# Siverteh/semantic-slam-master

Measured on AMD Instinct MI355X. Metric: frames/sec extract+match on TUM 640x480; match-index bit-exact vs CPU ref, higher is better.
Workload: dtype f32

## Files before the change

semantic-slam-master_amd/csrc/match.hip:

```cpp
#include "common.h"

namespace {

constexpr int QB = 128;
constexpr int CB = 64;
constexpr int NTM = 256;

template <int ROWS, int D>
struct Stager {
    static constexpr int GL = D == 128 ? 4 : 5, GM = D / 8 - 1, LDD = D + 4;
    static constexpr int ITEMS = ROWS * (D / 8) / NTM;
    float4 lo[ITEMS], hi[ITEMS];
    bool ok[ITEMS];
    __device__ __forceinline__ void load(const float *__restrict__ src, int first, int n_valid, int tid) {
#pragma unroll
        for (int i = 0; i < ITEMS; i++) {
            const int it = tid + NTM * i, row = it >> GL, g = it & GM;
            ok[i] = first + row < n_valid;
            const float4 *p = reinterpret_cast<const float4 *>(src + (long long)(ok[i] ? first + row : 0) * D + 8 * g);
            lo[i] = p[0];
            hi[i] = p[1];
        }
    }
    __device__ __forceinline__ void store(float *dst, int tid) const {
#pragma unroll
        for (int i = 0; i < ITEMS; i++) {
            const int it = tid + NTM * i, row = it >> GL, g = it & GM;
            float4 ev, od;
            const bool k = ok[i];
            kp8_split(make_float4(k ? lo[i].x : 0.f, k ? lo[i].y : 0.f, k ? lo[i].z : 0.f, k ? lo[i].w : 0.f),
                      make_float4(k ? hi[i].x : 0.f, k ? hi[i].y : 0.f, k ? hi[i].z : 0.f, k ? hi[i].w : 0.f), ev, od);
            *reinterpret_cast<float4 *>(dst + row * LDD + 8 * g) = ev;
            *reinterpret_cast<float4 *>(dst + row * LDD + 8 * g + 4) = od;
        }
    }
};

__device__ __forceinline__ unsigned long long sim_key(float v, float qoff, unsigned nqi) {
    unsigned u = __float_as_uint(v + qoff);
    u ^= (unsigned)((int)u >> 31) | 0x80000000u;
    return ((unsigned long long)u << 32) | nqi;
}

struct RowBest {
    float best, second;
    int besti, li;
};
template <int STEP, int CT, bool ONEPASS, bool MASKED, bool SECOND>
__device__ __forceinline__ void red_step(const f32x16 &acc, int sbase, int nc, int r, int h, float qoff, unsigned nqi, RowBest &rb,
                                         unsigned long long (&k)[8], unsigned long long &kk, int &jj) {
    if constexpr (STEP < 8) {
        if constexpr (STEP == 0 && CT == 0) rb.li = -1;
#pragma unroll
        for (int e = 2 * STEP; e < 2 * STEP + 2; e++) {
            const int lit = 32 * CT + (e & 3) + 8 * (e >> 2);
            float v = acc[e];
            if constexpr (MASKED) v = sbase + lit + 4 * h < nc ? v : -INFINITY;
            const bool gt = v > rb.best;
            if constexpr (SECOND) rb.second = __builtin_amdgcn_fmed3f(v, rb.best, rb.second);
            rb.li = gt ? lit : rb.li;
            rb.best = gt ? v : rb.best;
        }
        if constexpr (STEP == 7 && CT == 1) rb.besti = rb.li >= 0 ? sbase + 4 * h + rb.li : rb.besti;
    } else if constexpr (!ONEPASS) {
    } else if constexpr (STEP < 16) {
        constexpr int i = STEP - 8;
        typedef unsigned u32x2 __attribute__((ext_vector_type(2)));
        const unsigned long long lo = sim_key(acc[i], qoff, nqi), hi = sim_key(acc[i + 8], qoff, nqi);
        const u32x2 w0 = __builtin_amdgcn_permlane16_swap((unsigned)lo, (unsigned)hi, false, false);
        const u32x2 w1 = __builtin_amdgcn_permlane16_swap((unsigned)(lo >> 32), (unsigned)(hi >> 32), false, false);
        const unsigned long long a = ((unsigned long long)w1[0] << 32) | w0[0], b = ((unsigned long long)w1[1] << 32) | w0[1];
        k[i] = a > b ? a : b;
    } else if constexpr (STEP < 23) {
        constexpr int m = STEP < 20 ? 4 : (STEP < 22 ? 2 : 1);
        constexpr int i = STEP < 20 ? STEP - 16 : (STEP < 22 ? STEP - 20 : 0);
        const bool up = (r & (2 * m)) != 0;
        unsigned long long lo = k[i], hi = k[i + m];
        asm("" : "+v"(lo), "+v"(hi));
        const unsigned long long keep = up ? hi : lo, send = up ? lo : hi;
        const unsigned long long o = __shfl_xor(send, 2 * m);
        k[i] = keep > o ? keep : o;
    } else {
        const unsigned long long o = __shfl_xor(k[0], 1);
        kk = k[0] > o ? k[0] : o;
        jj = sbase + 32 * CT + crow((r >> 1) & 15, h);
    }
}
template <int FIRST, int N, bool ONEPASS, bool MASKED, bool SECOND>
__device__ __forceinline__ void red_steps(const f32x16 (&acc)[2], int s, int nc, int r, int h, float qoff, unsigned nqi, RowBest &rb,
                                          unsigned long long (&k)[2][8], unsigned long long (&kk)[2], int (&jj)[2]) {
    if constexpr (N > 0) {
        constexpr int ct = FIRST / 24;
        red_step<FIRST % 24, ct, ONEPASS, MASKED, SECOND>(acc[ct], s * CB, nc, r, h, qoff, nqi, rb, k[ct], kk[ct], jj[ct]);
        red_steps<FIRST + 1, N - 1, ONEPASS, MASKED, SECOND>(acc, s, nc, r, h, qoff, nqi, rb, k, kk, jj);
    }
}

struct StridedPairs {
    __device__ __forceinline__ bool frames(long long p, long long &f1, long long &f2) const {
        f1 = f2 = p;
        return true;
    }
    static __device__ __forceinline__ bool unwritten(unsigned long long) { return false; }
};
struct ListedPairs {
    const int *first, *second;
    int n_bank;
    __device__ __forceinline__ bool frames(long long p, long long &f1, long long &f2) const {
        const int a = first[p], b = second[p];
        if ((unsigned)a >= (unsigned)n_bank || (unsigned)b >= (unsigned)n_bank) return false;
        f1 = a;
        f2 = b;
        return true;
    }
    static __device__ __forceinline__ bool unwritten(unsigned long long key) { return key == 0ull; }
};

template <int D, bool ONEPASS, bool SECOND, class PAIRS>
__global__ __launch_bounds__(NTM, D == 128 ? 2 : 1) void sim_argmax_kernel(const float *__restrict__ desc1, long long stride1, int n1,
                                                            const float *__restrict__ desc2, long long stride2, int n2,
                                                            int *__restrict__ nn12, float *__restrict__ s12,
                                                            int *__restrict__ nn21, float *__restrict__ s21,
                                                            float *__restrict__ second12,
                                                            unsigned long long *__restrict__ keys, int n_pairs, int qblocks,
                                                            PAIRS pairs) {
    constexpr int LDD = D + 4;
    __shared__ __attribute__((aligned(16))) float Cs[2 * CB * LDD];
    const int tid = threadIdx.x, lane = tid & 63, wave = tid >> 6, r = lane & 31, h = lane >> 5;
    const int dir = blockIdx.y;
    const int xcd = blockIdx.x & 7, slot = blockIdx.x >> 3;
    const long long pair = (long long)(slot / qblocks) * 8 + xcd;
    if (pair >= n_pairs) return;
    long long f1, f2;
    if (!pairs.frames(pair, f1, f2)) {
        const int i = (slot % qblocks) * QB + tid;
        if (tid < QB && i < (dir == 0 ? n1 : n2)) {
            (dir == 0 ? nn12 + pair * n1 : nn21 + pair * n2)[i] = 0;
            float *val = dir == 0 ? s12 : s21;
            if (val) val[pair * (dir == 0 ? n1 : n2) + i] = 0.0f;
            if (dir == 0 && second12) second12[pair * n1 + i] = 0.0f;
        }
        return;
    }
    const float *q = dir == 0 ? desc1 + f1 * stride1 : desc2 + f2 * stride2;
    const float *c = dir == 0 ? desc2 + f2 * stride2 : desc1 + f1 * stride1;
    const int nq = dir == 0 ? n1 : n2, nc = dir == 0 ? n2 : n1;
    const int q0 = (slot % qblocks) * QB;
    if (q0 >= nq) return;
    int *o_idx = (dir == 0 ? nn12 + pair * n1 : nn21 + pair * n2);
    float *o_val = dir == 0 ? (s12 ? s12 + pair * n1 : nullptr) : (s21 ? s21 + pair * n2 : nullptr);
    float *o_sec = (dir == 0 && second12) ? second12 + pair * n1 : nullptr;

    Stager<CB, D> sc;
    sc.load(c, 0, nc, tid);
    const int qi = q0 + wave * 32 + r;
    const bool qok = qi < nq;
    float qreg[D / 2];
    {
        const float4 *qp = reinterpret_cast<const float4 *>(q + (long long)(qok ? qi : 0) * D);
        const float qm = qok ? 1.0f : 0.0f;
#pragma unroll
        for (int i = 0; i < D / 4; i++) {
            const float4 v = qp[i];
            qreg[2 * i] = (h ? v.y : v.x) * qm;
            qreg[2 * i + 1] = (h ? v.w : v.z) * qm;
        }
    }
    sc.store(Cs, tid);
    __syncthreads();

    RowBest rb = {-INFINITY, -INFINITY, 0x7fffffff, -1};
    const float qoff = qok ? 0.0f : -INFINITY;
    const unsigned nqi = ~(unsigned)qi;
    const int nstage = (nc + CB - 1) / CB;

#define M1_MMA(g_, A_, acc_)                                                                                          \
    {                                                                                                                 \
                    \
        const f32x4 a0 = *reinterpret_cast<const f32x4 *>((A_) + 8 * (g_));                                          \
        const f32x4 a1 = *reinterpret_cast<const f32x4 *>((A_) + 32 * LDD + 8 * (g_));                                \
        _Pragma("unroll") for (int st = 0; st < 4; st++) {                                                            \
            acc_[0] = mfma32(a0[st], qreg[4 * (g_) + st], acc_[0]);                                                   \
            acc_[1] = mfma32(a1[st], qreg[4 * (g_) + st], acc_[1]);                                                   \
        }                                                                                                             \
    }
    auto commit = [&](const unsigned long long (&kk)[2], const int (&jj)[2]) {
        if (ONEPASS) {
#pragma unroll
            for (int ct = 0; ct < 2; ct++)
                if (!(r & 1) && jj[ct] < nc) atomicMax(keys + pair * n2 + jj[ct], kk[ct]);
        }
    };

    f32x16 held[2];
#pragma unroll
    for (int e = 0; e < 16; e++) held[0][e] = held[1][e] = 0.0f;
    {
        const float *A = Cs + r * LDD + 4 * h;
#pragma unroll
        for (int g = 0; g < D / 8; g++) M1_MMA(g, A, held)
    }
    if (nstage > 1) {
        sc.load(c, CB, nc, tid);
        sc.store(Cs + CB * LDD, tid);
    }
    __syncthreads();
    unsigned long long kq[2][8];
    for (int s = 1; s < nstage; s++) {
        if (s + 1 < nstage) sc.load(c, (s + 1) * CB, nc, tid);
        const float *A = Cs + (s & 1) * CB * LDD + r * LDD + 4 * h;
        f32x16 acc[2];
        unsigned long long kk[2] = {0ull, 0ull};
        int jj[2] = {0, 0};
#pragma unroll
        for (int e = 0; e < 16; e++) acc[0][e] = acc[1][e] = 0.0f;
#define M1_SLOT(g_)                                                                                                   \
        _Pragma("unroll") for (int u = 0; u < D / 128; u++) M1_MMA((D / 128) * (g_) + u, A, acc)                       \
        __builtin_amdgcn_sched_barrier(0);                                                                            \
        red_steps<3 * (g_), 3, ONEPASS, false, SECOND>(held, s - 1, nc, r, h, qoff, nqi, rb, kq, kk, jj);                              \
        __builtin_amdgcn_sched_barrier(0);
        M1_SLOT(0) M1_SLOT(1) M1_SLOT(2) M1_SLOT(3) M1_SLOT(4) M1_SLOT(5) M1_SLOT(6) M1_SLOT(7)
        M1_SLOT(8) M1_SLOT(9) M1_SLOT(10) M1_SLOT(11) M1_SLOT(12) M1_SLOT(13) M1_SLOT(14) M1_SLOT(15)
#undef M1_SLOT
        held[0] = acc[0];
        held[1] = acc[1];
        if (s + 1 < nstage) sc.store(Cs + ((s + 1) & 1) * CB * LDD, tid);
        __builtin_amdgcn_sched_barrier(0);
        commit(kk, jj);
        __syncthreads();
    }
#undef M1_MMA
    {
        unsigned long long kk[2] = {0ull, 0ull};
        int jj[2] = {0, 0};
        red_steps<0, 48, ONEPASS, true, SECOND>(held, nstage - 1, nc, r, h, qoff, nqi, rb, kq, kk, jj);
        commit(kk, jj);
    }
    float best = rb.best, second = rb.second;
    int besti = rb.besti;
    {
        const float ov = __shfl_xor(best, 32), os = __shfl_xor(second, 32);
        const int oi = __shfl_xor(besti, 32);
        if (ov > best || (ov == best && oi < besti)) {
            second = fmaxf(best, os);
            best = ov;
            besti = oi;
        } else {
            second = fmaxf(second, ov);
        }
    }
    if (h == 0 && qok) {
        o_idx[qi] = (unsigned)besti < (unsigned)nc ? besti : 0;
        if (o_val) o_val[qi] = best;
        if (o_sec) o_sec[qi] = second;
    }
}

template <class PAIRS>
__global__ __launch_bounds__(256) void keys_decode_kernel(const unsigned long long *__restrict__ keys, long long n, int n1,
                                                           int *__restrict__ nn21, float *__restrict__ s21) {
    const long long i = (long long)blockIdx.x * 256 + threadIdx.x;
    if (i >= n) return;
    const unsigned long long kk = keys[i];
    if (PAIRS::unwritten(kk)) {
        nn21[i] = 0;
        if (s21) s21[i] = 0.0f;
        return;
    }
    unsigned u = (unsigned)(kk >> 32);
    u ^= (u >> 31) ? 0x80000000u : 0xffffffffu;
    const unsigned qi = ~(unsigned)kk;
    nn21[i] = qi < (unsigned)n1 ? (int)qi : 0;
    if (s21) s21[i] = __uint_as_float(u);
}

template <class PAIRS>
__global__ __launch_bounds__(256) void match_finalize_kernel(const int *__restrict__ nn12, const float *__restrict__ s12,
                                                              const int *__restrict__ nn21, int n1, int n2,
                                                              const float *__restrict__ sc1, long long ss1,
                                                              const float *__restrict__ sc2, long long ss2,
                                                              const float *__restrict__ in1, const float *__restrict__ in2,
                                                              float w_desc, float w_sal, float t_sal, float t_sim,
                                                              float t_int, long long *__restrict__ matches,
                                                              float *__restrict__ quality, int *__restrict__ count, PAIRS pairs) {
    __shared__ int wave_tot[4];
    __shared__ int running;
    const int tid = threadIdx.x, lane = tid & 63, wave = tid >> 6;
    const long long p = blockIdx.x;
    long long f1, f2;
    if (!pairs.frames(p, f1, f2)) {
        if (tid == 0) count[p] = 0;
        for (int sl = tid; sl < n1; sl += 256) {
            matches[(p * n1 + sl) * 2] = 0;
            matches[(p * n1 + sl) * 2 + 1] = 0;
            quality[p * n1 + sl] = 0.f;
        }
        return;
    }
    nn12 += p * n1;
    s12 += p * n1;
    nn21 += p * n2;
    sc1 += f1 * ss1;
    sc2 += f2 * ss2;
    if (in1) in1 += f1 * ss1;
    if (in2) in2 += f2 * ss2;
    matches += p * n1 * 2;
    quality += p * n1;
    if (tid == 0) running = 0;
    __syncthreads();
    for (int base = 0; base < n1; base += 256) {
        const int i = base + tid;
        bool ok = false;
        int j = 0;
        float sim = 0.f, avg = 0.f;
        if (i < n1) {
            j = nn12[i];
            if ((unsigned)j < (unsigned)n2 && nn21[j] == i) {
                sim = s12[i];
                avg = (sc1[i] + sc2[j]) / 2.0f;
                ok = (avg >= t_sal) && (sim >= t_sim);
                if (in1 && in2) ok = ok && ((in1[i] + in2[j]) / 2.0f >= t_int);
            }
        }
        int inc = ok ? 1 : 0;
#pragma unroll
        for (int off = 1; off < 64; off <<= 1) {
            const int t = __shfl_up(inc, off);
            if (lane >= off) inc += t;
        }
        if (lane == 63) wave_tot[wave] = inc;
        __syncthreads();
        int off0 = running;
        for (int w = 0; w < wave; w++) off0 += wave_tot[w];
        if (ok) {
            const int slot = off0 + inc - 1;
            matches[2 * slot] = i;
            matches[2 * slot + 1] = j;
            quality[slot] = w_desc * sim + w_sal * avg;
        }
        __syncthreads();
        if (tid == 0) running += wave_tot[0] + wave_tot[1] + wave_tot[2] + wave_tot[3];
        __syncthreads();
    }
    if (tid == 0) count[p] = running;
    for (int sl = running + tid; sl < n1; sl += 256) {
        matches[2 * sl] = 0;
        matches[2 * sl + 1] = 0;
        quality[sl] = 0.f;
    }
}

template <class PAIRS>
__global__ __launch_bounds__(256) void match_finalize_rule_kernel(const int *__restrict__ nn12, const float *__restrict__ s12,
                                                                   const float *__restrict__ second12, const int *__restrict__ nn21,
                                                                   int n1, int n2, int rule, float param,
                                                                   long long *__restrict__ matches, float *__restrict__ value,
                                                                   int *__restrict__ count, PAIRS pairs) {
    __shared__ int wave_tot[4];
    __shared__ int running;
    const int tid = threadIdx.x, lane = tid & 63, wave = tid >> 6;
    const long long p = blockIdx.x;
    long long f1, f2;
    if (!pairs.frames(p, f1, f2)) {
        if (tid == 0) count[p] = 0;
        for (int sl = tid; sl < n1; sl += 256) {
            matches[(p * n1 + sl) * 2] = 0;
            matches[(p * n1 + sl) * 2 + 1] = 0;
            value[p * n1 + sl] = 0.f;
        }
        return;
    }
    nn12 += p * n1;
    s12 += p * n1;
    if (second12) second12 += p * n1;
    if (nn21) nn21 += p * n2;
    matches += p * n1 * 2;
    value += p * n1;
    if (tid == 0) running = 0;
    __syncthreads();
    for (int base = 0; base < n1; base += 256) {
        const int i = base + tid;
        bool ok = false;
        int j = 0;
        float val = 0.f;
        if (i < n1) {
            j = nn12[i];
            if ((unsigned)j < (unsigned)n2) {
                const float best = s12[i];
                if (rule == SSLAM_RULE_TRACKED) {
                    ok = best > param;
                    val = best;
                } else if (nn21[j] == i) {
                    const float sec = second12[i];
                    if (rule == SSLAM_RULE_RATIO_BEST) {
                        ok = best > fmaxf(sec, -1.0f) * param;
                        val = best;
                    } else {
                        ok = __fdiv_rn(sec, __fadd_rn(best, 1e-8f)) < param;
                        val = __fsub_rn(1.0f, best);
                    }
                }
            }
        }
        int inc = ok ? 1 : 0;
#pragma unroll
        for (int off = 1; off < 64; off <<= 1) {
            const int t = __shfl_up(inc, off);
            if (lane >= off) inc += t;
        }
        if (lane == 63) wave_tot[wave] = inc;
        __syncthreads();
        int off0 = running;
        for (int w = 0; w < wave; w++) off0 += wave_tot[w];
        if (ok) {
            const int slot = off0 + inc - 1;
            matches[2 * slot] = i;
            matches[2 * slot + 1] = j;
            value[slot] = val;
        }
        __syncthreads();
        if (tid == 0) running += wave_tot[0] + wave_tot[1] + wave_tot[2] + wave_tot[3];
        __syncthreads();
    }
    if (tid == 0) count[p] = running;
    for (int sl = running + tid; sl < n1; sl += 256) {
        matches[2 * sl] = 0;
        matches[2 * sl + 1] = 0;
        value[sl] = 0.f;
    }
}

}

extern "C" long long sslam_sim_argmax_workspace_bytes(int n2, int n_pairs) {
    if (n2 <= 0 || n_pairs <= 0) return SSLAM_E_INVALID;
    const int forced = (int)sslam_knob(KNOB_M1_VARIANT, 0);
    if (forced == 1 || (forced == 0 && n_pairs < 16)) return 0;
    return (long long)n_pairs * n2 * (long long)sizeof(unsigned long long);
}

template <int D, class PAIRS>
static int launch_sim_argmax(const float *desc1, long long stride1, int n1, const float *desc2, long long stride2, int n2, int n_pairs,
                             int32_t *nn12, float *s12, int32_t *nn21, float *s21, float *second12, void *workspace,
                             long long workspace_bytes, void *stream, PAIRS pairs) {
    if ((long long)n_pairs * ((((n1 > n2 ? n1 : n2) + QB - 1) / QB)) > 0x7ffffff0LL / 8) return SSLAM_E_UNSUPPORTED;
    const int forced = (int)sslam_knob(KNOB_M1_VARIANT, 0);
    hipStream_t st = (hipStream_t)stream;
    const long long need = (long long)n_pairs * n2 * (long long)sizeof(unsigned long long);
    const bool have_ws = workspace && workspace_bytes >= need;
    if (forced == 2 && !have_ws) return SSLAM_E_INVALID;
    if (have_ws && (forced == 2 || (forced == 0 && n_pairs >= 16))) {
        unsigned long long *keys = (unsigned long long *)workspace;
        if (hipMemsetAsync(keys, 0, (size_t)need, st) != hipSuccess) return SSLAM_E_LAUNCH;
        const int qb1 = (n1 + QB - 1) / QB;
        const dim3 grid((unsigned)((n_pairs + 7) / 8 * 8 * qb1), 1, 1);
        if (second12)
            hipLaunchKernelGGL((sim_argmax_kernel<D, true, true, PAIRS>), grid, dim3(NTM), 0, st, desc1, stride1, n1, desc2, stride2, n2, nn12,
                               s12, nn21, s21, second12, keys, n_pairs, qb1, pairs);
        else
            hipLaunchKernelGGL((sim_argmax_kernel<D, true, false, PAIRS>), grid, dim3(NTM), 0, st, desc1, stride1, n1, desc2, stride2, n2, nn12,
                               s12, nn21, s21, second12, keys, n_pairs, qb1, pairs);
        SSLAM_CHECK_LAUNCH();
        const long long n = (long long)n_pairs * n2;
        hipLaunchKernelGGL(keys_decode_kernel<PAIRS>, dim3((unsigned)((n + 255) / 256)), dim3(256), 0, st, keys, n, n1, nn21, s21);
        SSLAM_CHECK_LAUNCH();
        return SSLAM_OK;
    }
    const int nmax = n1 > n2 ? n1 : n2;
    const int qbm = (nmax + QB - 1) / QB;
    const dim3 grid((unsigned)((n_pairs + 7) / 8 * 8 * qbm), 2, 1);
    if (second12)
        hipLaunchKernelGGL((sim_argmax_kernel<D, false, true, PAIRS>), grid, dim3(NTM), 0, st, desc1, stride1, n1, desc2, stride2, n2, nn12, s12,
                           nn21, s21, second12, nullptr, n_pairs, qbm, pairs);
    else
        hipLaunchKernelGGL((sim_argmax_kernel<D, false, false, PAIRS>), grid, dim3(NTM), 0, st, desc1, stride1, n1, desc2, stride2, n2, nn12, s12,
                           nn21, s21, second12, nullptr, n_pairs, qbm, pairs);
    SSLAM_CHECK_LAUNCH();
    return SSLAM_OK;
}

#define SSLAM_BY_WIDTH(d_, call128_, call256_) ((d_) == 128 ? (call128_) : (d_) == 256 ? (call256_) : SSLAM_E_UNSUPPORTED)

extern "C" int sslam_sim_argmax_ws_d(const float *desc1, long long stride1, int n1, const float *desc2, long long stride2,
                                     int n2, int n_pairs, int32_t *nn12, float *s12, int32_t *nn21, float *s21, float *second12,
                                     void *workspace, long long workspace_bytes, int d, void *stream) {
    if (!desc1 || !desc2 || !nn12 || !nn21 || n1 <= 0 || n2 <= 0 || n_pairs <= 0) return SSLAM_E_INVALID;
    if (((uintptr_t)desc1 | (uintptr_t)desc2) & 15 || (stride1 & 3) || (stride2 & 3) || ((uintptr_t)workspace & 7)) return SSLAM_E_INVALID;
    if (sslam_misaligned(4, nn12, s12, nn21, s21, second12)) return SSLAM_E_INVALID;
    return SSLAM_BY_WIDTH(d,
                          launch_sim_argmax<128>(desc1, stride1, n1, desc2, stride2, n2, n_pairs, nn12, s12, nn21, s21, second12, workspace,
                                                 workspace_bytes, stream, StridedPairs{}),
                          launch_sim_argmax<256>(desc1, stride1, n1, desc2, stride2, n2, n_pairs, nn12, s12, nn21, s21, second12, workspace,
                                                 workspace_bytes, stream, StridedPairs{}));
}
extern "C" int sslam_sim_argmax_ws(const float *desc1, long long stride1, int n1, const float *desc2, long long stride2,
                                   int n2, int n_pairs, int32_t *nn12, float *s12, int32_t *nn21, float *s21, float *second12,
                                   void *workspace, long long workspace_bytes, void *stream) {
    return sslam_sim_argmax_ws_d(desc1, stride1, n1, desc2, stride2, n2, n_pairs, nn12, s12, nn21, s21, second12, workspace,
                                 workspace_bytes, SSLAM_D, stream);
}

extern "C" int sslam_sim_argmax_pairs_d(const float *bank, long long frame_stride, int n_bank, int K, const int32_t *pair_first,
                                        const int32_t *pair_second, int n_pairs, int32_t *nn12, float *s12, int32_t *nn21, float *s21,
                                        float *second12, void *workspace, long long workspace_bytes, int d, void *stream) {
    if (!bank || !pair_first || !pair_second || !nn12 || !nn21 || n_bank <= 0 || K <= 0 || n_pairs <= 0) return SSLAM_E_INVALID;
    if (((uintptr_t)bank & 15) || (frame_stride & 3) || ((uintptr_t)workspace & 7) || (((uintptr_t)pair_first | (uintptr_t)pair_second) & 3))
        return SSLAM_E_INVALID;
    if (sslam_misaligned(4, nn12, s12, nn21, s21, second12)) return SSLAM_E_INVALID;
    const ListedPairs lp{pair_first, pair_second, n_bank};
    return SSLAM_BY_WIDTH(d,
                          launch_sim_argmax<128>(bank, frame_stride, K, bank, frame_stride, K, n_pairs, nn12, s12, nn21, s21, second12,
                                                 workspace, workspace_bytes, stream, lp),
                          launch_sim_argmax<256>(bank, frame_stride, K, bank, frame_stride, K, n_pairs, nn12, s12, nn21, s21, second12,
                                                 workspace, workspace_bytes, stream, lp));
}
extern "C" int sslam_sim_argmax_pairs(const float *bank, long long frame_stride, int n_bank, int K, const int32_t *pair_first,
                                      const int32_t *pair_second, int n_pairs, int32_t *nn12, float *s12, int32_t *nn21, float *s21,
                                      float *second12, void *workspace, long long workspace_bytes, void *stream) {
    return sslam_sim_argmax_pairs_d(bank, frame_stride, n_bank, K, pair_first, pair_second, n_pairs, nn12, s12, nn21, s21, second12,
                                    workspace, workspace_bytes, SSLAM_D, stream);
}

extern "C" int sslam_sim_argmax_d(const float *desc1, long long stride1, int n1, const float *desc2, long long stride2,
                                  int n2, int n_pairs, int32_t *nn12, float *s12, int32_t *nn21, float *s21, float *second12,
                                  int d, void *stream) {
    return sslam_sim_argmax_ws_d(desc1, stride1, n1, desc2, stride2, n2, n_pairs, nn12, s12, nn21, s21, second12, nullptr, 0, d, stream);
}
extern "C" int sslam_sim_argmax(const float *desc1, long long stride1, int n1, const float *desc2, long long stride2,
                                int n2, int n_pairs, int32_t *nn12, float *s12, int32_t *nn21, float *s21, float *second12,
                                void *stream) {
    return sslam_sim_argmax_ws_d(desc1, stride1, n1, desc2, stride2, n2, n_pairs, nn12, s12, nn21, s21, second12, nullptr, 0, SSLAM_D,
                                 stream);
}

extern "C" int sslam_match_finalize(const int32_t *nn12, const float *s12, const int32_t *nn21, int n1, int n2, int n_pairs,
                                    const float *scores1, long long sstride1, const float *scores2, long long sstride2,
                                    const float *intensity1, const float *intensity2, float w_desc, float w_sal,
                                    float min_saliency, float min_sim, float min_intensity, int64_t *matches,
                                    float *quality, int32_t *count, void *stream) {
    if (!nn12 || !s12 || !nn21 || !scores1 || !scores2 || !matches || !quality || !count || n1 <= 0 || n2 <= 0 ||
        n_pairs <= 0)
        return SSLAM_E_INVALID;
    if (sslam_misaligned(4, nn12, s12, nn21, scores1, scores2, intensity1, intensity2, quality, count) || sslam_misaligned(8, matches))
        return SSLAM_E_INVALID;
    hipLaunchKernelGGL(match_finalize_kernel<StridedPairs>, dim3(n_pairs), dim3(256), 0, (hipStream_t)stream, nn12, s12, nn21, n1, n2,
                       scores1, sstride1, scores2, sstride2, intensity1, intensity2, w_desc, w_sal, min_saliency, min_sim,
                       min_intensity, (long long *)matches, quality, count, StridedPairs{});
    SSLAM_CHECK_LAUNCH();
    return SSLAM_OK;
}

extern "C" int sslam_match_finalize_pairs(const int32_t *nn12, const float *s12, const int32_t *nn21, int K, int n_bank,
                                          const int32_t *pair_first, const int32_t *pair_second, int n_pairs, const float *scores_bank,
                                          long long score_stride, const float *intensity_bank, float w_desc, float w_sal,
                                          float min_saliency, float min_sim, float min_intensity, int64_t *matches, float *quality,
                                          int32_t *count, void *stream) {
    if (!nn12 || !s12 || !nn21 || !pair_first || !pair_second || !scores_bank || !matches || !quality || !count || K <= 0 ||
        n_bank <= 0 || n_pairs <= 0)
        return SSLAM_E_INVALID;
    if (((uintptr_t)pair_first | (uintptr_t)pair_second) & 3) return SSLAM_E_INVALID;
    if (sslam_misaligned(4, nn12, s12, nn21, scores_bank, intensity_bank, quality, count) || sslam_misaligned(8, matches)) return SSLAM_E_INVALID;
    hipLaunchKernelGGL(match_finalize_kernel<ListedPairs>, dim3(n_pairs), dim3(256), 0, (hipStream_t)stream, nn12, s12, nn21, K, K,
                       scores_bank, score_stride, scores_bank, score_stride, intensity_bank, intensity_bank, w_desc, w_sal,
                       min_saliency, min_sim, min_intensity, (long long *)matches, quality, count,
                       ListedPairs{pair_first, pair_second, n_bank});
    SSLAM_CHECK_LAUNCH();
    return SSLAM_OK;
}

template <int D, class PAIRS>
static int launch_sim_argmax_rows(const float *desc1, long long stride1, int n1, const float *desc2, long long stride2, int n2, int n_pairs,
                                  int32_t *nn12, float *s12, float *second12, void *stream, PAIRS pairs) {
    const int qb1 = (n1 + QB - 1) / QB;
    if ((long long)n_pairs * qb1 > 0x7ffffff0LL / 8) return SSLAM_E_UNSUPPORTED;
    const dim3 grid((unsigned)((n_pairs + 7) / 8 * 8 * qb1), 1, 1);
    hipStream_t st = (hipStream_t)stream;
    if (second12)
        hipLaunchKernelGGL((sim_argmax_kernel<D, false, true, PAIRS>), grid, dim3(NTM), 0, st, desc1, stride1, n1, desc2, stride2, n2, nn12, s12,
                           nullptr, nullptr, second12, nullptr, n_pairs, qb1, pairs);
    else
        hipLaunchKernelGGL((sim_argmax_kernel<D, false, false, PAIRS>), grid, dim3(NTM), 0, st, desc1, stride1, n1, desc2, stride2, n2, nn12, s12,
                           nullptr, nullptr, second12, nullptr, n_pairs, qb1, pairs);
    SSLAM_CHECK_LAUNCH();
    return SSLAM_OK;
}

extern "C" int sslam_sim_argmax_rows_d(const float *desc1, long long stride1, int n1, const float *desc2, long long stride2, int n2,
                                       int n_pairs, int32_t *nn12, float *s12, float *second12, int d, void *stream) {
    if (!desc1 || !desc2 || !nn12 || n1 <= 0 || n2 <= 0 || n_pairs <= 0) return SSLAM_E_INVALID;
    if (((uintptr_t)desc1 | (uintptr_t)desc2) & 15 || (stride1 & 3) || (stride2 & 3)) return SSLAM_E_INVALID;
    if (sslam_misaligned(4, nn12, s12, second12)) return SSLAM_E_INVALID;
    return SSLAM_BY_WIDTH(d,
                          launch_sim_argmax_rows<128>(desc1, stride1, n1, desc2, stride2, n2, n_pairs, nn12, s12, second12, stream, StridedPairs{}),
                          launch_sim_argmax_rows<256>(desc1, stride1, n1, desc2, stride2, n2, n_pairs, nn12, s12, second12, stream, StridedPairs{}));
}
extern "C" int sslam_sim_argmax_rows(const float *desc1, long long stride1, int n1, const float *desc2, long long stride2, int n2,
                                     int n_pairs, int32_t *nn12, float *s12, float *second12, void *stream) {
    return sslam_sim_argmax_rows_d(desc1, stride1, n1, desc2, stride2, n2, n_pairs, nn12, s12, second12, SSLAM_D, stream);
}

extern "C" int sslam_sim_argmax_rows_pairs_d(const float *bank, long long frame_stride, int n_bank, int K, const int32_t *pair_first,
                                             const int32_t *pair_second, int n_pairs, int32_t *nn12, float *s12, float *second12,
                                             int d, void *stream) {
    if (!bank || !pair_first || !pair_second || !nn12 || n_bank <= 0 || K <= 0 || n_pairs <= 0) return SSLAM_E_INVALID;
    if (((uintptr_t)bank & 15) || (frame_stride & 3) || (((uintptr_t)pair_first | (uintptr_t)pair_second) & 3)) return SSLAM_E_INVALID;
    if (sslam_misaligned(4, nn12, s12, second12)) return SSLAM_E_INVALID;
    const ListedPairs lp{pair_first, pair_second, n_bank};
    return SSLAM_BY_WIDTH(d,
                          launch_sim_argmax_rows<128>(bank, frame_stride, K, bank, frame_stride, K, n_pairs, nn12, s12, second12, stream, lp),
                          launch_sim_argmax_rows<256>(bank, frame_stride, K, bank, frame_stride, K, n_pairs, nn12, s12, second12, stream, lp));
}
extern "C" int sslam_sim_argmax_rows_pairs(const float *bank, long long frame_stride, int n_bank, int K, const int32_t *pair_first,
                                           const int32_t *pair_second, int n_pairs, int32_t *nn12, float *s12, float *second12,
                                           void *stream) {
    return sslam_sim_argmax_rows_pairs_d(bank, frame_stride, n_bank, K, pair_first, pair_second, n_pairs, nn12, s12, second12, SSLAM_D,
                                         stream);
}

static bool rule_args_ok(const int32_t *nn12, const float *s12, const float *second12, const int32_t *nn21, int n1, int n2, int n_pairs,
                         int rule, const int64_t *matches, const float *value, const int32_t *count) {
    if (!nn12 || !s12 || !matches || !value || !count || n1 <= 0 || n2 <= 0 || n_pairs <= 0) return false;
    if (rule != SSLAM_RULE_RATIO_BEST && rule != SSLAM_RULE_RATIO_SECOND && rule != SSLAM_RULE_TRACKED) return false;
    if (rule != SSLAM_RULE_TRACKED && (!second12 || !nn21)) return false;
    if (sslam_misaligned(4, nn12, s12, second12, nn21, value, count) || sslam_misaligned(8, matches)) return false;
    return rule != SSLAM_RULE_RATIO_SECOND || n2 >= 2;
}

extern "C" int sslam_match_finalize_rule(const int32_t *nn12, const float *s12, const float *second12, const int32_t *nn21, int n1,
                                         int n2, int n_pairs, int rule, float param, int64_t *matches, float *value, int32_t *count,
                                         void *stream) {
    if (!rule_args_ok(nn12, s12, second12, nn21, n1, n2, n_pairs, rule, matches, value, count)) return SSLAM_E_INVALID;
    hipLaunchKernelGGL(match_finalize_rule_kernel<StridedPairs>, dim3(n_pairs), dim3(256), 0, (hipStream_t)stream, nn12, s12, second12, nn21,
                       n1, n2, rule, param, (long long *)matches, value, count, StridedPairs{});
    SSLAM_CHECK_LAUNCH();
    return SSLAM_OK;
}

extern "C" int sslam_match_finalize_rule_pairs(const int32_t *nn12, const float *s12, const float *second12, const int32_t *nn21, int K,
                                               int n_bank, const int32_t *pair_first, const int32_t *pair_second, int n_pairs, int rule,
                                               float param, int64_t *matches, float *value, int32_t *count, void *stream) {
    if (!rule_args_ok(nn12, s12, second12, nn21, K, K, n_pairs, rule, matches, value, count) || !pair_first || !pair_second || n_bank <= 0)
        return SSLAM_E_INVALID;
    if (((uintptr_t)pair_first | (uintptr_t)pair_second) & 3) return SSLAM_E_INVALID;
    hipLaunchKernelGGL(match_finalize_rule_kernel<ListedPairs>, dim3(n_pairs), dim3(256), 0, (hipStream_t)stream, nn12, s12, second12, nn21,
                       K, K, rule, param, (long long *)matches, value, count, ListedPairs{pair_first, pair_second, n_bank});
    SSLAM_CHECK_LAUNCH();
    return SSLAM_OK;
}
```

Baseline: 59920.

## Route column argmax through per-wave LDS transpose instead of cross-lane shuffles

The one-pass column (reverse-direction) argmax now writes each MFMA accumulator tile into a small per-wave LDS patch and reads it back transposed. Each lane scans 8 query values serially, and two DPP quad exchanges finish the reduction. This replaces the permlane16 swaps and the chain of 64-bit shfl_xor butterflies. The costs are extra LDS traffic and shared memory per block, plus a different committing-lane pattern, and bit-exact tie-breaking depends on the packed index key.

```diff
diff --git a/semantic-slam-master_amd/csrc/match.hip b/semantic-slam-master_amd/csrc/match.hip
--- a/semantic-slam-master_amd/csrc/match.hip
+++ b/semantic-slam-master_amd/csrc/match.hip
@@ -36,19 +36,77 @@
     }
 };
 
-__device__ __forceinline__ unsigned long long sim_key(float v, float qoff, unsigned nqi) {
-    unsigned u = __float_as_uint(v + qoff);
+__device__ __forceinline__ unsigned long long sim_key(float v, unsigned nqi) {
+    unsigned u = __float_as_uint(v + 0.0f);
     u ^= (unsigned)((int)u >> 31) | 0x80000000u;
     return ((unsigned long long)u << 32) | nqi;
+}
+
+struct ColLane {
+    float *w0, *w1;
+    const float *ra, *rb;
+    unsigned nq8;
+    int nvalid;
+    int jrow;
+    bool full;
+    __device__ __forceinline__ ColLane(float *patch, int lane, int qwave, int nq) {
+        const int r = lane & 31, h = lane >> 5, g = lane & 3, row = lane >> 2, sw = (row & 2) << 1;
+        w0 = patch + 256 * h + r;
+        w1 = patch + 256 * h + (r ^ 4);
+        ra = patch + 32 * row + ((8 * g) ^ sw);
+        rb = patch + 32 * row + ((8 * g + 4) ^ sw);
+        nq8 = ~(unsigned)(qwave + 8 * g);
+        nvalid = nq - (qwave + 8 * g);
+        jrow = 16 * (g & 1) + ((row & 3) + 8 * ((row >> 2) & 1) + 4 * (row >> 3));
+        full = __builtin_amdgcn_readfirstlane(qwave) + 32 <= nq;
+    }
+};
+template <int CTRL>
+__device__ __forceinline__ unsigned long long quad_key(unsigned long long k) {
+    const unsigned lo = __builtin_amdgcn_update_dpp(0u, (unsigned)k, CTRL, 0xf, 0xf, true);
+    const unsigned hi = __builtin_amdgcn_update_dpp(0u, (unsigned)(k >> 32), CTRL, 0xf, 0xf, true);
+    return ((unsigned long long)hi << 32) | lo;
 }
 
 struct RowBest {
     float best, second;
     int besti, li;
 };
+struct ColTile {
+    float v[8];
+    unsigned long long k0;
+};
+template <int H>
+__device__ __forceinline__ void col_store(const f32x16 &acc, const ColLane &cl) {
+#pragma unroll
+    for (int e = 0; e < 8; e++) ((e & 2) ? cl.w1 : cl.w0)[32 * ((e & 3) + 4 * (e >> 2))] = acc[8 * H + e];
+}
+__device__ __forceinline__ void col_load(ColTile &t, const ColLane &cl) {
+    const f32x4 a = *reinterpret_cast<const f32x4 *>(cl.ra), b = *reinterpret_cast<const f32x4 *>(cl.rb);
+#pragma unroll
+    for (int i = 0; i < 4; i++) {
+        t.v[i] = a[i];
+        t.v[4 + i] = b[i];
+    }
+}
+__device__ __forceinline__ unsigned long long col_scan(ColTile &t, const ColLane &cl) {
+    if (!cl.full) {
+#pragma unroll
+        for (int i = 0; i < 8; i++) t.v[i] = i < cl.nvalid ? t.v[i] : -INFINITY;
+    }
+    float best = t.v[0];
+    unsigned pos = 0;
+#pragma unroll
+    for (int i = 1; i < 8; i++) {
+        const bool gt = t.v[i] > best;
+        pos = gt ? i : pos;
+        best = gt ? t.v[i] : best;
+    }
+    return sim_key(best, cl.nq8 - pos);
+}
 template <int STEP, int CT, bool ONEPASS, bool MASKED, bool SECOND>
-__device__ __forceinline__ void red_step(const f32x16 &acc, int sbase, int nc, int r, int h, float qoff, unsigned nqi, RowBest &rb,
-                                         unsigned long long (&k)[8], unsigned long long &kk, int &jj) {
+__device__ __forceinline__ void red_step(const f32x16 &acc, int sbase, int nc, int h, const ColLane &cl, RowBest &rb, ColTile &t,
+                                         unsigned long long &kk, int &jj) {
     if constexpr (STEP < 8) {
         if constexpr (STEP == 0 && CT == 0) rb.li = -1;
 #pragma unroll
@@ -63,36 +121,32 @@
         }
         if constexpr (STEP == 7 && CT == 1) rb.besti = rb.li >= 0 ? sbase + 4 * h + rb.li : rb.besti;
     } else if constexpr (!ONEPASS) {
-    } else if constexpr (STEP < 16) {
-        constexpr int i = STEP - 8;
-        typedef unsigned u32x2 __attribute__((ext_vector_type(2)));
-        const unsigned long long lo = sim_key(acc[i], qoff, nqi), hi = sim_key(acc[i + 8], qoff, nqi);
-        const u32x2 w0 = __builtin_amdgcn_permlane16_swap((unsigned)lo, (unsigned)hi, false, false);
-        const u32x2 w1 = __builtin_amdgcn_permlane16_swap((unsigned)(lo >> 32), (unsigned)(hi >> 32), false, false);
-        const unsigned long long a = ((unsigned long long)w1[0] << 32) | w0[0], b = ((unsigned long long)w1[1] << 32) | w0[1];
-        k[i] = a > b ? a : b;
-    } else if constexpr (STEP < 23) {
-        constexpr int m = STEP < 20 ? 4 : (STEP < 22 ? 2 : 1);
-        constexpr int i = STEP < 20 ? STEP - 16 : (STEP < 22 ? STEP - 20 : 0);
-        const bool up = (r & (2 * m)) != 0;
-        unsigned long long lo = k[i], hi = k[i + m];
-        asm("" : "+v"(lo), "+v"(hi));
-        const unsigned long long keep = up ? hi : lo, send = up ? lo : hi;
-        const unsigned long long o = __shfl_xor(send, 2 * m);
-        k[i] = keep > o ? keep : o;
-    } else {
-        const unsigned long long o = __shfl_xor(k[0], 1);
-        kk = k[0] > o ? k[0] : o;
-        jj = sbase + 32 * CT + crow((r >> 1) & 15, h);
+    } else if constexpr (STEP == 8) {
+        col_store<0>(acc, cl);
+    } else if constexpr (STEP == 9 || STEP == 15) {
+        col_load(t, cl);
+    } else if constexpr (STEP == 12) {
+        t.k0 = col_scan(t, cl);
+        col_store<1>(acc, cl);
+    } else if constexpr (STEP == 18) {
+        const unsigned long long k1 = col_scan(t, cl);
+        const bool odd = (cl.jrow & 16) != 0;
+        const unsigned long long keep = odd ? k1 : t.k0, send = odd ? t.k0 : k1;
+        const unsigned long long o = quad_key<0xB1>(send);
+        t.k0 = keep > o ? keep : o;
+    } else if constexpr (STEP == 19) {
+        const unsigned long long o = quad_key<0x4E>(t.k0);
+        kk = t.k0 > o ? t.k0 : o;
+        jj = sbase + 32 * CT + cl.jrow;
     }
 }
 template <int FIRST, int N, bool ONEPASS, bool MASKED, bool SECOND>
-__device__ __forceinline__ void red_steps(const f32x16 (&acc)[2], int s, int nc, int r, int h, float qoff, unsigned nqi, RowBest &rb,
-                                          unsigned long long (&k)[2][8], unsigned long long (&kk)[2], int (&jj)[2]) {
+__device__ __forceinline__ void red_steps(const f32x16 (&acc)[2], int s, int nc, int h, const ColLane &cl, RowBest &rb, ColTile &t,
+                                          unsigned long long (&kk)[2], int (&jj)[2]) {
     if constexpr (N > 0) {
         constexpr int ct = FIRST / 24;
-        red_step<FIRST % 24, ct, ONEPASS, MASKED, SECOND>(acc[ct], s * CB, nc, r, h, qoff, nqi, rb, k[ct], kk[ct], jj[ct]);
-        red_steps<FIRST + 1, N - 1, ONEPASS, MASKED, SECOND>(acc, s, nc, r, h, qoff, nqi, rb, k, kk, jj);
+        red_step<FIRST % 24, ct, ONEPASS, MASKED, SECOND>(acc[ct], s * CB, nc, h, cl, rb, t, kk[ct], jj[ct]);
+        red_steps<FIRST + 1, N - 1, ONEPASS, MASKED, SECOND>(acc, s, nc, h, cl, rb, t, kk, jj);
     }
 }
 
@@ -126,6 +180,7 @@
                                                             PAIRS pairs) {
     constexpr int LDD = D + 4;
     __shared__ __attribute__((aligned(16))) float Cs[2 * CB * LDD];
+    __shared__ __attribute__((aligned(16))) float Ts[ONEPASS ? NTM / 64 * 512 : 4];
     const int tid = threadIdx.x, lane = tid & 63, wave = tid >> 6, r = lane & 31, h = lane >> 5;
     const int dir = blockIdx.y;
     const int xcd = blockIdx.x & 7, slot = blockIdx.x >> 3;
@@ -170,8 +225,7 @@
     __syncthreads();
 
     RowBest rb = {-INFINITY, -INFINITY, 0x7fffffff, -1};
-    const float qoff = qok ? 0.0f : -INFINITY;
-    const unsigned nqi = ~(unsigned)qi;
+    const ColLane cl(Ts + (ONEPASS ? 512 * wave : 0), lane, q0 + wave * 32, nq);
     const int nstage = (nc + CB - 1) / CB;
 
 #define M1_MMA(g_, A_, acc_)                                                                                          \
@@ -188,7 +242,7 @@
         if (ONEPASS) {
 #pragma unroll
             for (int ct = 0; ct < 2; ct++)
-                if (!(r & 1) && jj[ct] < nc) atomicMax(keys + pair * n2 + jj[ct], kk[ct]);
+                if ((lane & 3) < 2 && jj[ct] < nc) atomicMax(keys + pair * n2 + jj[ct], kk[ct]);
         }
     };
 
@@ -205,7 +259,7 @@
         sc.store(Cs + CB * LDD, tid);
     }
     __syncthreads();
-    unsigned long long kq[2][8];
+    ColTile ctile;
     for (int s = 1; s < nstage; s++) {
         if (s + 1 < nstage) sc.load(c, (s + 1) * CB, nc, tid);
         const float *A = Cs + (s & 1) * CB * LDD + r * LDD + 4 * h;
@@ -217,7 +271,7 @@
 #define M1_SLOT(g_)                                                                                                   \
         _Pragma("unroll") for (int u = 0; u < D / 128; u++) M1_MMA((D / 128) * (g_) + u, A, acc)                       \
         __builtin_amdgcn_sched_barrier(0);                                                                            \
-        red_steps<3 * (g_), 3, ONEPASS, false, SECOND>(held, s - 1, nc, r, h, qoff, nqi, rb, kq, kk, jj);                              \
+        red_steps<3 * (g_), 3, ONEPASS, false, SECOND>(held, s - 1, nc, h, cl, rb, ctile, kk, jj);                              \
         __builtin_amdgcn_sched_barrier(0);
         M1_SLOT(0) M1_SLOT(1) M1_SLOT(2) M1_SLOT(3) M1_SLOT(4) M1_SLOT(5) M1_SLOT(6) M1_SLOT(7)
         M1_SLOT(8) M1_SLOT(9) M1_SLOT(10) M1_SLOT(11) M1_SLOT(12) M1_SLOT(13) M1_SLOT(14) M1_SLOT(15)
@@ -233,7 +287,7 @@
     {
         unsigned long long kk[2] = {0ull, 0ull};
         int jj[2] = {0, 0};
-        red_steps<0, 48, ONEPASS, true, SECOND>(held, nstage - 1, nc, r, h, qoff, nqi, rb, kq, kk, jj);
+        red_steps<0, 48, ONEPASS, true, SECOND>(held, nstage - 1, nc, h, cl, rb, ctile, kk, jj);
         commit(kk, jj);
     }
     float best = rb.best, second = rb.second;
```

New measurement: 60080, median of 6. About the same (+0.3%).
